# mcveanlab/mccortex

Hardware: AMD Instinct MI355X
Metric: k-mers/s inserted (build), k=31, 50M x 150bp synthetic reads (higher is better)
Workload: dtype u64

## Files before the change

### mccortex_amd/csrc/mcx_defer.h

```cpp
#pragma once
#include "mcx_kernels.h"

namespace mcx {

enum : int { BIN_OWNER = 0, BIN_GROUP = 1, BIN_SUBLOCAL = 2, BIN_GLOBAL = 3 };

struct BinSpec {
  int mode;
  uint32_t nparts;
  uint32_t nlocal;
  uint32_t rep;
  uint32_t nout;
  uint32_t seg_mod;
  uint32_t lb1;
  uint32_t region0;
};

__device__ __forceinline__ uint32_t out_seg(const BinSpec &bs, uint32_t ob0, uint32_t b)
{
  if (bs.mode == BIN_GLOBAL)
    return ((((b >> bs.lb1) * bs.rep + blockIdx.x % bs.rep) << bs.lb1) | (b & ((1u << bs.lb1) - 1u)));
  return ob0 + b;
}

struct BinOut {
  uint64_t *keys;
  uint8_t *edges;
  unsigned long long *counts;
  uint64_t cap;
  uint64_t *ov_keys;
  uint8_t *ov_edges;
  unsigned long long *ov_counts;
  uint64_t ov_cap;
};

#define MCX_LDS_AS __attribute__((address_space(3)))

#ifdef MCX_PHASES
__device__ unsigned long long g_phase[3][8];
#define MCX_PH_DECL unsigned long long ph_t = wall_clock64(), ph_acc[8] = {0, 0, 0, 0, 0, 0, 0, 0};
#define MCX_PH(i) { const unsigned long long n_ = wall_clock64(); ph_acc[i] += n_ - ph_t; ph_t = n_; }
#define MCX_PH_COUNT ph_acc[7]++;
#define MCX_PH_DUMP(kid) { if (threadIdx.x == 0) for (int i_ = 0; i_ < 8; i_++) atomicAdd(&g_phase[kid][i_], ph_acc[i_]); }
#else
#define MCX_PH_DECL
#define MCX_PH(i)
#define MCX_PH_COUNT
#define MCX_PH_DUMP(kid)
#endif
constexpr int kMaxBins = 2048;
constexpr uint64_t kQMask = (1ull << 56) - 1;

template <int W> __device__ __forceinline__ Kmer<W> tuple_pack(const Kmer<W> &q, uint32_t e)
{
  Kmer<W> t = q;
  t.w[0] |= (uint64_t)e << 56;
  return t;
}
template <int W> __device__ __forceinline__ Kmer<W> tuple_q(const Kmer<W> &t)
{
  Kmer<W> q = t;
  q.w[0] &= kQMask;
  return q;
}

constexpr int kRounds = 2;
constexpr int kStage = kTile / kRounds;

template <int T_, int TILE_, int R_ = kRounds> struct Geo {
  static constexpr int kT = T_, kTileG = TILE_, kRoundsG = R_, kStageG = TILE_ / R_;
};
using Geo256 = Geo<kThreads, kTile>;

template <int W, int NB, bool FULL, class G = Geo256> struct BinLds {
  using geo = G;
  uint64_t skey[G::kStageG * W];
  unsigned long long gbase[NB];
  uint32_t cnt[NB + 64];
  uint32_t rnk[NB + 64];
  uint32_t off[NB + 64];
  uint32_t wsum[G::kT / 64];
  uint16_t sbin[G::kStageG];
  uint8_t se[FULL ? G::kStageG : 16];
};

__device__ __forceinline__ uint32_t tid_now()
{
  uint32_t t = threadIdx.x;
  asm volatile("" : "+v"(t));
  return t;
}

template <int NB, int T = kThreads> struct BinRes { unsigned long long g0[(NB + T - 1) / T]; };

template <class LDS, int NB>
__device__ __forceinline__ void bin_reserve(LDS &L, const BinSpec &bs, const BinOut &out, uint32_t ob0, BinRes<NB, LDS::geo::kT> &res,
                                            bool trash_beyond = false)
{
  constexpr int kT = LDS::geo::kT;
  const int tid = threadIdx.x;
  __syncthreads();
  {
    constexpr int PERB = NB / kT;
    static_assert(NB % kT == 0, "bins per thread");
    uint32_t c[PERB], x = 0;
#pragma unroll
    for (int i = 0; i < PERB; i++) {
      const uint32_t b = (uint32_t)tid * PERB + i;
      c[i] = b < bs.nlocal ? L.cnt[b] : 0;
      x += c[i];
    }
    const uint32_t mine = x;
#pragma unroll
    for (int d = 1; d < 64; d <<= 1) {
      const uint32_t y = __shfl_up(x, d, 64);
      if ((tid & 63) >= d) x += y;
    }
    if ((tid & 63) == 63) L.wsum[tid >> 6] = x;
    __syncthreads();
    uint32_t before = 0, total = 0;
#pragma unroll
    for (int w = 0; w < kT / 64; w++) {
      const uint32_t ws = L.wsum[w];
      if (w < (tid >> 6)) before += ws;
      total += ws;
    }
    uint32_t o = before + x - mine;
#pragma unroll
    for (int i = 0; i < PERB; i++) {
      const uint32_t b = (uint32_t)tid * PERB + i;
      if (b < bs.nlocal) L.off[b] = o;
      o += c[i];
    }
    if (tid < 64) L.off[bs.nlocal + tid] = tid && trash_beyond ? (uint32_t)LDS::geo::kTileG : total;
  }
  __syncthreads();
#pragma unroll
  for (int q = 0; q < (NB + kT - 1) / kT; q++) {
    const uint32_t b = (uint32_t)q * kT + tid;
    res.g0[q] = 0;
    if (b < bs.nlocal) {
      const uint32_t c = L.cnt[b];
      if (c) res.g0[q] = atomicAdd(&out.counts[out_seg(bs, ob0, b)], (unsigned long long)c);
    }
  }
}

constexpr unsigned long long kDstMask = (1ULL << 48) - 1;

template <class LDS, int NB>
__device__ __forceinline__ void bin_commit(LDS &L, const BinSpec &bs, const BinOut &out, uint32_t ob0, const BinRes<NB, LDS::geo::kT> &res)
{
  constexpr int kT = LDS::geo::kT;
#pragma unroll
  for (int q = 0; q < (NB + kT - 1) / kT; q++) {
    const uint32_t b = (uint32_t)q * kT + threadIdx.x;
    if (b < bs.nlocal) {
      const uint32_t o0 = L.off[b], o1 = L.off[b + 1];
      const unsigned long long g0 = res.g0[q];
      const unsigned long long room = out.cap > g0 ? out.cap - g0 : 0;
      const uint32_t lim = o0 + (uint32_t)min((unsigned long long)(o1 - o0), room);
      const unsigned long long dst = ((unsigned long long)out_seg(bs, ob0, b) * out.cap + g0 - o0) & kDstMask;
      L.gbase[b] = dst | ((unsigned long long)lim << 48);
    }
  }
}

template <class LDS> __device__ __forceinline__ uint32_t bin_rank(LDS &L, uint32_t local)
{
  return L.off[local] + atomicAdd(&L.rnk[local], 1u);
}

template <int W, bool FULL, class LDS>
__device__ __forceinline__ void bin_place(LDS &L, int round, uint32_t p, uint32_t local, const Kmer<W> &t, uint32_t e)
{
  constexpr uint32_t kSt = LDS::geo::kStageG;
  if ((int)(p / kSt) != round) return;
  const uint32_t q = p % kSt;
  L.skey[q * W] = t.w[0];
  if (W == 2) L.skey[q * W + 1] = t.w[W - 1];
  L.sbin[q] = (uint16_t)local;
  if (FULL) L.se[q] = (uint8_t)e;
}

template <int W, bool ONECOL, bool FULL, int SH, class LDS>
__device__ __forceinline__ void bin_writeout(LDS &L, int round, const BinSpec &bs, const BinOut &out, uint32_t ob0,
                                             uint32_t region_of_seg, const InsertSink<W, ONECOL> &isink,
                                             uint32_t &novel, uint32_t &full)
{
  __syncthreads();
  const uint32_t n = L.off[bs.nlocal];
  constexpr uint32_t kSt = LDS::geo::kStageG;
  const uint32_t lo = (uint32_t)round * kSt;
  const uint32_t hi = min(n, lo + kSt);
  auto emit = [&](uint32_t p, uint32_t b, unsigned long long gb, uint64_t t0, uint64_t t1) {
    if (p < (uint32_t)(gb >> 48)) {
      const uint64_t at = (gb + p) & kDstMask;
      uint64_t *kd = out.keys + at * W;
      kd[0] = t0;
      if (W == 2) kd[1] = t1;
      if (FULL) out.edges[at] = L.se[p - lo];
    } else if (FULL || bs.mode == BIN_OWNER) {
      full = 2;
    } else {
      Kmer<W> tq;
      tq.w[0] = t0;
      if (W == 2) tq.w[W - 1] = t1;
      const uint32_t e = (uint32_t)(tq.w[0] >> 56);
      const Kmer<W> qq = tuple_q<W>(tq);
      const uint32_t lbq = lbq_of(isink.t);
      if (SH == 2) {
        const Kmer<W> key = key_unquot<W>(qq, lbq, b ^ mix_g(region_mix<W>(qq), lbq));
        const uint32_t owner = b >> bs.lb1;
        const unsigned long long pos = atomicAdd(&out.ov_counts[owner], 1ULL);
        if (pos < out.ov_cap) {
          uint64_t *kd = out.ov_keys + ((uint64_t)owner * out.ov_cap + pos) * W;
          kd[0] = key.w[0];
          if (W == 2) kd[1] = key.w[W - 1];
          out.ov_edges[(uint64_t)owner * out.ov_cap + pos] = (uint8_t)e;
        } else {
          const unsigned long long sp_cap = bs.region0 ? out.ov_counts[bs.nparts + 1] : 0;
          const unsigned long long sp = sp_cap ? atomicAdd(&out.ov_counts[bs.nparts], 1ULL) : 0;
          if (sp < sp_cap) {
            const uint64_t at = (uint64_t)bs.nparts * out.ov_cap + sp;
            uint64_t *kd = out.ov_keys + at * W;
            kd[0] = key.w[0];
            if (W == 2) kd[1] = key.w[W - 1];
            out.ov_edges[at] = (uint8_t)e;
          } else {
            full = 2;
          }
        }
      } else {
        table_mark_written(isink.t);
        table_count_fallback(isink.t);
        const uint32_t region = bs.mode == BIN_GROUP ? b : region_of_seg;
        const Kmer<W> key = key_unquot<W>(qq, lbq, r_of<W>(isink.t, region, qq));
        const uint64_t slot = key_slot<W>(isink.t, key);
        const uint64_t cur = *key_ptr_t<W, ONECOL>(isink.t, slot);
        probe_insert<W, ONECOL>(isink.t, key, slot, cur, 0, e, isink.col, novel, full);
      }
    }
  };
  for (uint32_t p = lo + threadIdx.x; p < hi; p += LDS::geo::kT) {
    const uint32_t q = p - lo;
    const uint32_t b = L.sbin[q];
    emit(p, b, L.gbase[b], L.skey[q * W], W == 2 ? L.skey[q * W + W - 1] : 0);
  }
  if (round + 1 < LDS::geo::kRoundsG) __syncthreads();
}

struct LaneWin { uint32_t a2, a1, a0, r2, r1, r0; };
__device__ __forceinline__ uint32_t pairrev32(uint32_t x)
{
  const uint32_t r = __builtin_bitreverse32(x);
  return ((r >> 1) & 0x55555555u) | ((r & 0x55555555u) << 1);
}
__device__ __forceinline__ LaneWin lane_win(const uint32_t *s_code, uint32_t pl, int k)
{
  LaneWin w;
  w.a2 = s_code[pl >> 4];
  w.a1 = s_code[(pl >> 4) + 1];
  w.a0 = s_code[(pl >> 4) + 2];
  const uint32_t c2 = pairrev32(~w.a0), c1 = pairrev32(~w.a1), c0 = pairrev32(~w.a2);
  const int t = 66 - 2 * k;
  if (t < 32) {
    w.r2 = (c2 << t) | (c1 >> (32 - t));
    w.r1 = (c1 << t) | (c0 >> (32 - t));
    w.r0 = c0 << t;
  } else {
    const uint64_t x = (((uint64_t)c1 << 32) | c0) << (t - 32);
    w.r2 = (uint32_t)(x >> 32);
    w.r1 = (uint32_t)x;
    w.r0 = 0;
  }
  return w;
}

template <int W, bool ONECOL>
__device__ __noinline__ void foreign_insert(const InsertSink<W, ONECOL> &isink, Kmer<W> key, uint32_t e,
                                            uint32_t &novel, uint32_t &full)
{
  table_mark_written(isink.t);
  table_count_foreign(isink.t);
  const uint64_t slot = key_slot<W>(isink.t, key);
  const uint64_t cur = *key_ptr_t<W, ONECOL>(isink.t, slot);
  probe_insert<W, ONECOL>(isink.t, key, slot, cur, 0, e, isink.col, novel, full);
}

template <int W, bool ONECOL, int NB, bool FULL, int SH, bool PK, int T = kThreads>
__global__ __launch_bounds__(T, (W == 1 ? 4 : 3)) void k_stream_bin(StreamArgs a_arg, BinSpec bs, BinOut out_arg,
                                                                  InsertSink<W, ONECOL> isink_arg)
{
  constexpr int H = T / kThreads;
  static_assert(T == kThreads || (T == 2 * kThreads && !FULL), "256 threads, or 512 for packed bins");
  __shared__ uint32_t s_code_h[H][kChunks + 4];
  __shared__ uint32_t s_inv_h[H][kChunks / 2 + 4];
  struct Cold { StreamArgs a; InsertSink<W, ONECOL> isink; };
  __shared__ Cold cold;
  if (threadIdx.x == 0) { cold.a = a_arg; cold.isink = isink_arg; }
  __syncthreads();
  const StreamArgs &a = cold.a;
  const BinOut &out = out_arg;
  const InsertSink<W, ONECOL> &isink = cold.isink;
  const uint64_t a_tile0 = a_arg.tile0, a_ntiles = a_arg.ntiles;
  const uint32_t t_lb1 = isink_arg.t.lb1, t_lbq = isink_arg.t.lb1 + isink_arg.t.lbo, t_part = isink_arg.t.part;
  extern __shared__ __attribute__((aligned(16))) unsigned char dyn_lds[];
  using LDS = BinLds<W, NB, FULL, Geo<T, T * kPosPerLane>>;
  LDS &L = *reinterpret_cast<LDS *>(dyn_lds);

  const int tid0 = threadIdx.x & (kThreads - 1);
  const uint64_t half0 = (uint64_t)(threadIdx.x / kThreads);
  const int k = a_arg.k;
  uint32_t n_kmers = 0, n_contigs = 0, n_novel = 0, full = 0;
  const uint64_t top_mask = (W == 1) ? (~0ULL >> (64 - 2 * k)) : (~0ULL >> (128 - 2 * k));
  const int first_shift = (W == 1) ? (2 * k - 2) : (2 * k - 66);
  const uint32_t ob0 = (blockIdx.x % bs.rep) * bs.nout;

  TileSrc pre;
  pre.a = make_uint4(0, 0, 0, 0); pre.b = make_uint4(0, 0, 0, 0);
  {
    const uint64_t t0 = a_tile0 + (uint64_t)blockIdx.x * H + half0;
    if (t0 < a_ntiles) tile_fetch<PK>(a_arg, t0, tid0, pre);
  }
  MCX_PH_DECL
  for (uint64_t tile_b = a_tile0 + (uint64_t)blockIdx.x * H; tile_b < a_ntiles; tile_b += (uint64_t)gridDim.x * H) {
    const int tid_blk = (int)tid_now();
    const int tid = tid_blk & (kThreads - 1);
    const uint64_t tile = tile_b + (uint64_t)(tid_blk / kThreads);
    const bool have_tile = H == 1 || tile < a_ntiles;
    uint32_t *s_code = s_code_h[H == 1 ? 0 : tid_blk / kThreads];
    uint32_t *s_inv = s_inv_h[H == 1 ? 0 : tid_blk / kThreads];
    MCX_PH(6) MCX_PH_COUNT
    tile_stage<PK>(a_arg, pre, tid, s_code, s_inv);
    for (uint32_t b = tid_blk; b < bs.nlocal + 64; b += T) { L.cnt[b] = 0; L.rnk[b] = 0; }
    if (tid < 4) { s_code[kChunks + tid] = 0; s_inv[kChunks / 2 + tid] = 0xFFFFFFFFu; }
    {
      const uint64_t tn = tile + (uint64_t)gridDim.x * H;
      if (tn < a_ntiles) tile_fetch<PK>(a_arg, tn, tid, pre);
    }
    __syncthreads();
    MCX_PH(0)

    const uint32_t pl = 16u * (uint32_t)(tid + 1);
    const uint64_t Vh = inv_win64(s_inv, pl);
    const uint64_t Vl = (W == 2) ? inv_win64(s_inv, pl + 64) : 0;
    const uint32_t prev_chunk_inv = (s_inv[(pl - 1) >> 5] >> (31 - ((pl - 1) & 31))) & 1u;
    uint32_t range = have_tile ? 0xFFFFu : 0u;
    if (have_tile) {
      const uint64_t plo = a.pos_lo, phi = a.pos_hi, T0 = tile * kTile;
      if (T0 < plo || T0 + kTile > phi) {
        const uint64_t P0 = T0 + 16ull * (uint64_t)tid;
        const int j_lo = plo > P0 ? (int)min((uint64_t)kPosPerLane, plo - P0) : 0;
        const int j_hi = phi > P0 ? (int)min((uint64_t)kPosPerLane, phi - P0) : 0;
        range = ((0x10000u >> j_lo) - 1u) & ~((0x10000u >> j_hi) - 1u);
      }
    }
    uint32_t ok16, nok16, pok16;
    {
      uint64_t Mh = Vh, Ml = Vl;
      for (int c = 1; c < k;) {
        const int s = min(c, k - c);
        if (W == 2) Mh |= (Mh << s) | (Ml >> (64 - s));
        else Mh |= Mh << s;
        if (W == 2) Ml |= Ml << s;
        c += s;
      }
      ok16 = ~(uint32_t)(Mh >> 48) & range;
      const int sh = 112 - k;
      const uint64_t nx = sh >= 64 ? (Vh >> (sh - 64)) : ((Vh << (64 - sh)) | (W == 2 ? (Vl >> sh) : 0));
      nok16 = ~(uint32_t)nx & 0xFFFFu;
      pok16 = ~((prev_chunk_inv << 15) | (uint32_t)(Vh >> 49)) & 0xFFFFu;
    }

    Kmer<W> tk[kPosPerLane];
    uint32_t tle[kPosPerLane];
    const uint32_t trash = bs.nlocal + 1u + ((uint32_t)tid_blk & 31u);
    n_kmers += __popc(ok16);
    n_contigs += __popc(ok16 & ~pok16);
    {
      const uint32_t own = s_code[pl >> 4];
      const uint32_t before = s_code[(pl - 1) >> 4] & 3u;
      const uint32_t lbq = t_lbq;
      const uint32_t qmask = (1u << lbq) - 1u, lmask = (1u << t_lb1) - 1u;
      Kmer<W> fw, rc;
      uint64_t feed;
      LaneWin lw;
      if (W == 1) {
        lw = lane_win(s_code, pl, k);
        feed = code_win64(s_code, pl + (uint32_t)k);
      } else {
        const uint64_t hi = code_win64(s_code, pl), lo = code_win64(s_code, pl + 32);
        const int s = 128 - 2 * k;
        fw.w[0] = hi >> s;
        fw.w[W - 1] = (lo >> s) | (hi << (64 - s));
        rc = revcomp<W>(fw, k);
        feed = code_win64(s_code, pl + (uint32_t)k);
      }
      const uint32_t feed32 = (uint32_t)(feed >> 32);
      uint32_t arr_prev = 0;
      const uint32_t key_sh = 64u - 2u * (uint32_t)k;
      const uint32_t mix_sh = (32u - lbq) & 31u;
#pragma unroll
      for (int j = 0; j < kPosPerLane; j++) {
        const uint32_t prev_nuc = j == 0 ? before : ((own >> (32 - 2 * j)) & 3u);
        const uint32_t nuc_next = (feed32 >> (30 - 2 * j)) & 3u;
        const uint32_t valid = 0u - ((ok16 >> (15 - j)) & 1u);
        const uint32_t nb = (nok16 >> (15 - j)) & 1u, pb = (pok16 >> (15 - j)) & 1u;
        uint32_t o, local;
        Kmer<W> key;
        uint64_t sel = 0;
        if (W == 1) {
          const uint32_t fh = j ? __builtin_amdgcn_alignbit(lw.a2, lw.a1, 32 - 2 * j) : lw.a2;
          const uint32_t fl = j ? __builtin_amdgcn_alignbit(lw.a1, lw.a0, 32 - 2 * j) : lw.a1;
          const uint32_t rh = j < 15 ? __builtin_amdgcn_alignbit(lw.r2, lw.r1, 2 + 2 * j) : lw.r2;
          const uint32_t rl = j < 15 ? __builtin_amdgcn_alignbit(lw.r1, lw.r0, 2 + 2 * j) : lw.r1;
          const uint64_t f = ((uint64_t)fh << 32) | fl, r = ((uint64_t)rh << 32) | rl;
          o = f < r ? 0u : 1u;
          sel = f < r ? f : r;
          key.w[0] = sel >> key_sh;
        } else {
          key = canonical<W>(fw, rc, o);
        }
        const uint32_t o4 = o << 2;
        const uint32_t e = (nb << (nuc_next | o4)) | (pb << ((prev_nuc ^ 7u) ^ o4));
        if (FULL) {
          uint32_t h2;
          kmer_hash<W>(key, 0, &h2);
          local = owner_of(h2, bs.nparts);
          tk[j] = key;
          local = (local & valid) | (trash & ~valid);
          tle[j] = local | (e << 24);
        } else {
          uint32_t G;
          Kmer<W> q;
          if (W == 1) {
            const uint64_t kk = sel >> key_sh;
            q.w[0] = kk >> lbq;
            G = ((uint32_t)kk ^ (region_mix<W>(q) >> mix_sh)) & qmask;
          } else {
            uint32_t r;
            q = key_quot<W>(key, lbq, r);
            G = r ^ mix_g(region_mix<W>(q), lbq);
          }
          local = SH == 1 ? (G & lmask) : G;
          tk[j] = tuple_pack<W>(q, e);
          if (SH == 1 && valid && (G >> t_lb1) != t_part) {
            foreign_insert<W, ONECOL>(isink, key, e, n_novel, full);
            local = trash;
          }
          local = (local & valid) | (trash & ~valid);
          tle[j] = local;
        }
        const uint32_t arr_now = atomicAdd(&L.cnt[local], 1u);
        if (j > 0) { tle[j - 1] |= arr_prev << 12; asm volatile("" : "+v"(tle[j - 1])); }
        arr_prev = arr_now;
        if (j == kPosPerLane - 1) tle[j] |= arr_now << 12;
        if (W == 1) asm volatile("" : "+v"(tle[j]), "+v"(tk[j].w[0]));
        else asm volatile("" : "+v"(tle[j]), "+v"(tk[j].w[0]), "+v"(tk[j].w[W - 1]));
        if (W == 2) {
          fw.w[0] = ((fw.w[0] << 2) | (fw.w[W - 1] >> 62)) & top_mask;
          fw.w[W - 1] = (fw.w[W - 1] << 2) | nuc_next;
          rc.w[W - 1] = (rc.w[W - 1] >> 2) | (rc.w[0] << 62);
          rc.w[0] = (rc.w[0] >> 2) | ((uint64_t)(3u - nuc_next) << first_shift);
        }
      }
    }
    MCX_PH(1)
    BinRes<NB, T> res;
    bin_reserve<LDS, NB>(L, bs, out, ob0, res, !FULL);
    MCX_PH(2)
#pragma unroll
    for (int j = 0; j < kPosPerLane; j++) {
      tle[j] += L.off[tle[j] & 0xfffu] << 12;
      if ((j & 3) == 3) asm volatile("" : "+v"(tle[j - 3]), "+v"(tle[j - 2]), "+v"(tle[j - 1]), "+v"(tle[j]));
    }
    bin_commit<LDS, NB>(L, bs, out, ob0, res);
    MCX_PH(3)
    for (int round = 0; round < kRounds; round++) {
#pragma unroll
      for (int j = 0; j < kPosPerLane; j++)
        bin_place<W, FULL, LDS>(L, round, FULL ? (tle[j] >> 12) & 0xfffu : tle[j] >> 12, tle[j] & 0xfffu, tk[j], tle[j] >> 24);
      bin_writeout<W, ONECOL, FULL, SH, LDS>(L, round, bs, out, ob0, 0, isink, n_novel, full);
      if (round == 0) { MCX_PH(4) } else { MCX_PH(5) }
    }
  }
  MCX_PH_DUMP(0)

  block_add(&a.ctr->kmers, n_kmers);
  block_add(&a.ctr->contigs, n_contigs);
  block_add(&a.ctr->novel, n_novel);
  if (full == 1) a.ctr->full = 1;
  if (full == 2) a.ctr->bin_over = 1;
  if (a.flag && n_contigs) *a.flag = 1;
}

struct TupleIn {
  const uint64_t *keys;
  const uint8_t *edges;
  const unsigned long long *counts;
  uint64_t seg_cap;
  uint32_t nseg;
  uint32_t seg_group, seg_stride;
  uint32_t set_rep;
  uint8_t set_map[32];
};
__device__ __forceinline__ uint64_t tuple_seg_phys(const TupleIn &in, uint32_t seg)
{
  uint32_t q = seg / in.seg_group;
  if (in.set_rep) q = (uint32_t)in.set_map[q / in.set_rep] * in.set_rep + q % in.set_rep;
  return (uint64_t)q * in.seg_stride + seg % in.seg_group;
}

template <int W, bool ONECOL, int NB, bool IN_FULL, bool SHARD, int T = kThreads, int R = kRounds, int P = 16>
__global__ __launch_bounds__(T, (W == 1 || T > kThreads ? 4 : 3)) void k_tuples_bin(TupleIn in, BinSpec bs, BinOut out,
                                                                         InsertSink<W, ONECOL> isink_arg, Counters *ctr)
{
  extern __shared__ __attribute__((aligned(16))) unsigned char dyn_lds[];
  using LDS = BinLds<W, NB, false, Geo<T, T * P, R>>;
  constexpr int kThreads = T, kTile = T * P;
  LDS &L = *reinterpret_cast<LDS *>(dyn_lds);
  __shared__ InsertSink<W, ONECOL> isink;
  if (threadIdx.x == 0) isink = isink_arg;
  __syncthreads();
  const uint32_t t_spb = isink_arg.t.spb, t_lb1 = isink_arg.t.lb1, t_lbq = isink_arg.t.lb1 + isink_arg.t.lbo, t_part = isink_arg.t.part;
  const int tid = threadIdx.x;
  uint32_t n_novel = 0, full = 0;
  const uint64_t chunks_per_seg = (in.seg_cap + kTile - 1) / kTile;
  const bool xcd = bs.mode == BIN_SUBLOCAL && gridDim.x % 8 == 0 && bs.seg_mod % 8 == 0 && in.nseg % bs.seg_mod == 0;
  const uint32_t group = xcd ? blockIdx.x % 8 : 0;
  const uint32_t nseg_g = xcd ? in.nseg / 8 : in.nseg;
  constexpr uint32_t kWin = 2;
  const uint32_t bins_g = xcd ? bs.seg_mod / 8 : 1;
  const uint32_t reps = xcd ? in.nseg / bs.seg_mod : 1;
  const uint32_t win_segs = kWin * reps;
  const uint32_t nwin = (bins_g + kWin - 1) / kWin;
  const uint64_t nchunks = xcd ? (uint64_t)nwin * chunks_per_seg * win_segs : chunks_per_seg * nseg_g;
  const uint64_t v0 = xcd ? blockIdx.x / 8 : blockIdx.x, vstep = xcd ? gridDim.x / 8 : gridDim.x;
  const uint32_t lmask = (1u << t_lb1) - 1u;
  MCX_PH_DECL
  for (uint64_t v = v0; v < nchunks; v += vstep) {
    uint32_t seg;
    uint64_t start;
    if (xcd) {
      const uint64_t per_win = chunks_per_seg * win_segs;
      const uint32_t win = (uint32_t)(v / per_win);
      const uint64_t rem = v % per_win;
      const uint32_t s = (uint32_t)(rem % win_segs);
      const uint32_t rgi = win * kWin + s % kWin;
      if (rgi >= bins_g) continue;
      seg = (s / kWin) * bs.seg_mod + group + 8 * rgi;
      start = (rem / win_segs) * kTile;
    } else {
      seg = (uint32_t)(v % nseg_g);
      start = (v / nseg_g) * kTile;
    }
    const uint64_t pseg = tuple_seg_phys(in, seg);
    uint64_t cnt = in.counts ? (uint64_t)in.counts[pseg] : in.seg_cap;
    if (cnt > in.seg_cap) cnt = in.seg_cap;
    if (start >= cnt) continue;
    const uint32_t n = (uint32_t)min((uint64_t)kTile, cnt - start);
    const uint32_t lregion = bs.mode == BIN_SUBLOCAL ? seg % bs.seg_mod : 0;
    const uint32_t region = bs.region0 + lregion;
    const uint32_t ob0 = (bs.mode == BIN_SUBLOCAL ? lregion * t_spb : 0) + (blockIdx.x % bs.rep) * bs.nout;
    MCX_PH(6) MCX_PH_COUNT
    __syncthreads();
    for (uint32_t b = tid; b < bs.nlocal + 64; b += kThreads) { L.cnt[b] = 0; L.rnk[b] = 0; }
    __syncthreads();
    MCX_PH(0)
    const uint32_t trash = bs.nlocal + 1u + ((uint32_t)tid & 31u);
    const uint64_t *kin = in.keys + (pseg * in.seg_cap + start) * W;
    const uint8_t *ein = IN_FULL ? in.edges + pseg * in.seg_cap + start : nullptr;
    constexpr int PER = kTile / kThreads;
    Kmer<W> tk[PER];
    uint32_t ev[IN_FULL ? PER : 1], loc[PER];
    uint32_t okm = 0;
    const bool vec16 = !IN_FULL && (((uintptr_t)in.keys & 15u) == 0) && (W == 2 || (in.seg_cap & 1u) == 0);
    if (vec16) {
      const ulonglong2 *kin2 = reinterpret_cast<const ulonglong2 *>(kin);
#pragma unroll
      for (int q = 0; q < PER; q += (W == 1 ? 2 : 1)) {
        const uint32_t p = (uint32_t)(q / (W == 1 ? 2 : 1)) * kThreads + tid;
        const uint32_t i = W == 1 ? 2 * p : p;
        tk[q].w[0] = 0; tk[q + (W == 1 ? 1 : 0)].w[W - 1] = 0;
        if (i < n) {
          const ulonglong2 x = kin2[p];
          okm |= 1u << q;
          if (W == 1) {
            tk[q].w[0] = x.x;
            tk[q + (W == 1 ? 1 : 0)].w[0] = x.y;
            if (i + 1 < n) okm |= 2u << q;
          } else {
            tk[q].w[0] = x.x;
            tk[q].w[W - 1] = x.y;
          }
        }
      }
    } else {
#pragma unroll
    for (int q = 0; q < PER; q++) {
      const uint32_t i = (uint32_t)q * kThreads + tid;
      if (i < n) okm |= 1u << q;
      tk[q].w[0] = 0; if (W == 2) tk[q].w[W - 1] = 0;
      if (IN_FULL) ev[q] = 0;
      if (i < n) {
        tk[q].w[0] = kin[(uint64_t)i * W];
        if (W == 2) tk[q].w[W - 1] = kin[(uint64_t)i * W + 1];
        if (IN_FULL) ev[q] = ein[i];
      }
    }
    }
#pragma unroll
    for (int q = 0; q < PER; q++) {
      const uint32_t i = (uint32_t)q * kThreads + tid;
      uint32_t hb;
      if (IN_FULL) {
        uint32_t r;
        const uint32_t lbq = t_lbq;
        const Kmer<W> key = tk[q];
        const Kmer<W> qq = key_quot<W>(key, lbq, r);
        const uint32_t G = r ^ mix_g(region_mix<W>(qq), lbq);
        hb = 0;
        loc[q] = G & lmask;
// ... 436 lines not shown
```

### mccortex_amd/csrc/mcx_kernels.h

```cpp
#pragma once
#include <hip/hip_runtime.h>
#include <stdint.h>
#include "mcx_kmer.h"

namespace mcx {

constexpr int kBucket = 4;
template <int W> struct Sub {
  static constexpr int kShift = W == 1 ? 12 : 11;
  static constexpr uint64_t kSlots = 1ull << kShift;
  static constexpr uint32_t kBuckets = (uint32_t)(kSlots / kBucket);
};
__host__ __device__ constexpr int sub_shift_for_words(int W) { return W == 1 ? 12 : 11; }

struct TableView {
  uint64_t *rec;
  uint64_t nslots;
  uint64_t nmain;
  uint32_t lb1;
  uint32_t lbo;
  uint32_t part;
  uint32_t spb;
  uint32_t S;
  uint32_t max_probe;
// ... 389 lines not shown
      if (cv) __hip_atomic_fetch_add(val, (uint64_t)cv << 8, MCX_RLX, MCX_AGENT);
      if (e) __hip_atomic_fetch_or(val, (uint64_t)e, MCX_RLX, MCX_AGENT);
    }
    loaded++;
  }
  if (novel) { atomicAdd(&ctr->novel, (unsigned long long)novel); atomicAdd(&st->novel, (unsigned long long)novel); }
  if (loaded) atomicAdd(&st->loaded, (unsigned long long)loaded);
  if (full) ctr->full = 1;
}

template <int W>
__global__ __launch_bounds__(256) void k_record_keys(const uint8_t *recs, uint64_t n, uint32_t rec_bytes, uint64_t *k0, uint64_t *k1)
{
  const uint64_t i = (uint64_t)blockIdx.x * blockDim.x + threadIdx.x;
  if (i >= n) return;
  const uint8_t *p = recs + i * rec_bytes;
  k0[i] = (uint64_t)load_le32(p) | (uint64_t)load_le32(p + 4) << 32;
  if (W == 2) k1[i] = (uint64_t)load_le32(p + 8) | (uint64_t)load_le32(p + 12) << 32;
}

__global__ __launch_bounds__(256) void k_gather_records(const uint8_t *in, const uint64_t *perm, uint64_t n, uint32_t rec_bytes, uint8_t *out)
{
  const uint64_t i = ((uint64_t)blockIdx.x * blockDim.x + threadIdx.x) >> 4;
  const uint32_t l = threadIdx.x & 15u;
  if (i >= n) return;
  const uint8_t *src = in + perm[i] * rec_bytes;
  uint8_t *dst = out + i * rec_bytes;
  for (uint32_t b = l; b < rec_bytes; b += 16) dst[b] = src[b];
}

template <int W>
__global__ __launch_bounds__(256) void k_check_sorted(const uint64_t *k0, const uint64_t *k1, uint64_t n, unsigned long long *first_bad)
{
  const uint64_t i = (uint64_t)blockIdx.x * blockDim.x + threadIdx.x;
  if (i + 1 >= n) return;
  bool lt = k0[i] < k0[i + 1];
  if (W == 2 && k0[i] == k0[i + 1]) lt = k1[i] < k1[i + 1];
  if (!lt) atomicMin(first_bad, (unsigned long long)(i + 1));
}

__global__ __launch_bounds__(256) void k_covg_scan(TableView t, uint32_t ncols, unsigned long long *out,
                                                   unsigned long long *hist, uint32_t nbins, uint32_t lbins)
{
  extern __shared__ unsigned long long s_acc[];
  unsigned long long *s_hist = s_acc + 2 * ncols;
  for (uint32_t c = threadIdx.x; c < 2 * ncols + lbins; c += blockDim.x) s_acc[c] = 0;
  __syncthreads();
  for (uint64_t slot = (uint64_t)blockIdx.x * blockDim.x + threadIdx.x; slot < t.nslots; slot += (uint64_t)gridDim.x * blockDim.x) {
    const uint64_t *r = key_ptr(t, slot);
    uint64_t w0, v1 = 0;
    if (t.S == 2) {
      const ulonglong2 kv = *reinterpret_cast<const ulonglong2 *>(r);
      w0 = kv.x; v1 = kv.y;
    } else {
      w0 = r[0];
    }
    if (!(w0 & kFlag)) continue;
    uint64_t sum = 0;
    for (uint32_t c = 0; c < ncols; c++) {
      uint64_t cv = (t.S == 2 ? v1 : *val_ptr(t, slot, c)) >> 8;
      if (cv > 0xFFFFFFFFull) cv = 0xFFFFFFFFull;
      if (cv) { atomicAdd(&s_acc[c], 1ULL); atomicAdd(&s_acc[ncols + c], (unsigned long long)cv); }
      sum += cv;
    }
    if (sum > 0xFFFFFFFFull) sum = 0xFFFFFFFFull;
    if (hist) {
      const uint64_t bin = sum < nbins ? sum : nbins - 1;
      if (bin < lbins) atomicAdd(&s_hist[bin], 1ULL);
      else atomicAdd(&hist[bin], 1ULL);
    }
  }
  __syncthreads();
  for (uint32_t c = threadIdx.x; c < 2 * ncols; c += blockDim.x)
    if (s_acc[c]) atomicAdd(&out[c], s_acc[c]);
  for (uint32_t c = threadIdx.x; c < lbins; c += blockDim.x)
    if (s_hist[c]) atomicAdd(&hist[c], s_hist[c]);
}

template <int W, bool ONECOL> struct InsertSink {
  TableView t;
  uint32_t col;
};

constexpr int kThreads = 256;
constexpr int kPosPerLane = 16;
constexpr int kTile = kThreads * kPosPerLane;
constexpr int kChunks = 272;
constexpr int kBatch = 4;

struct StreamArgs {
  const uint8_t *stream;
  const uint32_t *code;
  const uint16_t *inv;
  uint64_t nbytes;
  uint64_t pos_lo, pos_hi;
  uint64_t tile0, ntiles;
  int k;
  Counters *ctr;
  unsigned char *flag;
};

__device__ __forceinline__ uint64_t code_win64(const uint32_t *s_code, uint32_t q)
{
  const uint32_t j = q >> 4, sh = (q & 15u) * 2u;
  const uint64_t hi = ((uint64_t)s_code[j] << 32) | s_code[j + 1];
  const uint64_t lo = s_code[j + 2];
  return sh ? (hi << sh) | (lo >> (32 - sh)) : hi;
}
__device__ __forceinline__ uint64_t inv_win64(const uint32_t *s_inv, uint32_t q)
{
  const uint32_t j = q >> 5, sh = q & 31u;
  const uint64_t hi = ((uint64_t)s_inv[j] << 32) | s_inv[j + 1];
  const uint64_t lo = s_inv[j + 2];
  return sh ? (hi << sh) | (lo >> (32 - sh)) : hi;
}

__device__ __forceinline__ uint4 load_chunk(const uint8_t *stream, uint64_t nbytes, int64_t g)
{
  if (g >= 0 && (uint64_t)g + 16 <= nbytes) return *reinterpret_cast<const uint4 *>(stream + g);
  uint32_t w[4] = {0, 0, 0, 0};
  if (g + 16 > 0 && g < (int64_t)nbytes)
    for (int i = 0; i < 16; i++) {
      const int64_t p = g + i;
      if (p >= 0 && (uint64_t)p < nbytes) w[i >> 2] |= (uint32_t)stream[p] << (8 * (i & 3));
    }
  return make_uint4(w[0], w[1], w[2], w[3]);
}

__device__ __forceinline__ void encode_words(const uint4 v, uint32_t &code, uint32_t &inv)
{
  const uint32_t w[4] = {v.x, v.y, v.z, v.w};
  code = 0; inv = 0;
#pragma unroll
  for (int i = 0; i < 4; i++) {
    const uint32_t x = w[i];
    const uint32_t t = ((x >> 1) ^ (x >> 2)) & 0x03030303u;
    code = (code << 8) | ((t * 0x40100401u) >> 24);
    const uint32_t u = x & 0xDFDFDFDFu;
#define MCX_NZ(v) ((((v) & 0x7F7F7F7Fu) + 0x7F7F7F7Fu) | (v))
    const uint32_t bad = MCX_NZ(u ^ 0x41414141u) & MCX_NZ(u ^ 0x43434343u) &
                         MCX_NZ(u ^ 0x47474747u) & MCX_NZ(u ^ 0x54545454u) & 0x80808080u;
#undef MCX_NZ
    inv = (inv << 4) | ((((bad >> 7) * 0x08040201u) >> 24) & 0xFu);
  }
}

__device__ __forceinline__ void encode_chunk(const uint8_t *stream, uint64_t nbytes, int64_t g,
                                             uint32_t &code, uint32_t &inv)
{
  encode_words(load_chunk(stream, nbytes, g), code, inv);
}

struct TileSrc { uint4 a, b; };
template <bool PK> __device__ __forceinline__ void tile_fetch(const StreamArgs &a, uint64_t tile, int tid, TileSrc &t)
{
  if (PK) {
    const int64_t c0 = (int64_t)(tile * (kTile / 16)) - 1;
    const int64_t nch = (int64_t)((a.nbytes + 15) / 16);
    const int64_t c = c0 + tid, c2 = c + kThreads;
    const bool in = c >= 0 && c < nch;
    t.a.x = in ? a.code[c] : 0u;
    t.a.y = in ? (uint32_t)a.inv[c] : 0xFFFFu;
    if (tid < kChunks - kThreads) {
      const bool in2 = c2 >= 0 && c2 < nch;
      t.b.x = in2 ? a.code[c2] : 0u;
      t.b.y = in2 ? (uint32_t)a.inv[c2] : 0xFFFFu;
    }
  } else {
    const int64_t r0 = (int64_t)(tile * kTile) - 16;
    t.a = load_chunk(a.stream, a.nbytes, r0 + 16 * (int64_t)tid);
    if (tid < kChunks - kThreads) t.b = load_chunk(a.stream, a.nbytes, r0 + 16 * (int64_t)(tid + kThreads));
  }
}
template <bool PK> __device__ __forceinline__ void tile_stage(const StreamArgs &a, const TileSrc &t, int tid, uint32_t *s_code, uint32_t *s_inv)
{
  uint32_t code, inv;
  (void)a;
  if (PK) { code = t.a.x; inv = t.a.y; } else encode_words(t.a, code, inv);
  s_code[tid] = code;
  reinterpret_cast<uint16_t *>(s_inv)[tid ^ 1] = (uint16_t)inv;
  if (tid < kChunks - kThreads) {
    if (PK) { code = t.b.x; inv = t.b.y; } else encode_words(t.b, code, inv);
    s_code[tid + kThreads] = code;
    reinterpret_cast<uint16_t *>(s_inv)[(tid + kThreads) ^ 1] = (uint16_t)inv;
  }
}

__global__ void k_pack_stream(const uint8_t *stream, uint64_t nbytes, uint32_t *code_out, uint16_t *inv_out)
{
  const uint64_t c = (uint64_t)blockIdx.x * blockDim.x + threadIdx.x;
  if (c * 16 >= nbytes) return;
  uint32_t code, inv;
  encode_words(load_chunk(stream, nbytes, (int64_t)(c * 16)), code, inv);
  code_out[c] = code;
  inv_out[c] = (uint16_t)inv;
}

template <int W> struct Occ {
  Kmer<W> key;
  uint32_t e;
};

template <int W, bool ONECOL>
__device__ __forceinline__ void flush_batch(const InsertSink<W, ONECOL> &sink, const Occ<W> (&occ)[kBatch],
                                            const bool (&ov)[kBatch], uint32_t &novel, uint32_t &full)
{
  uint64_t slot[kBatch], cur[kBatch], hint[kBatch];
#pragma unroll
  for (int i = 0; i < kBatch; i++) {
    cur[i] = 0; hint[i] = 0; slot[i] = 0;
    if (ov[i]) {
      slot[i] = key_slot<W>(sink.t, occ[i].key);
      const uint64_t *r = key_ptr_t<W, ONECOL>(sink.t, slot[i]);
      if (W == 1 && ONECOL) {
        const ulonglong2 kv = *reinterpret_cast<const ulonglong2 *>(r);
        cur[i] = kv.x; hint[i] = kv.y;
      } else {
        cur[i] = r[0];
      }
    }
  }
#pragma unroll
  for (int i = 0; i < kBatch; i++)
    if (ov[i]) probe_insert<W, ONECOL>(sink.t, occ[i].key, slot[i], cur[i], hint[i], occ[i].e, sink.col, novel, full);
}

__device__ __forceinline__ uint32_t owner_of(uint32_t h2, uint32_t nparts)
{
  return (uint32_t)(((uint64_t)h2 * nparts) >> 32);
}

__device__ __forceinline__ void lane_masks_wide(const uint32_t *s_inv, uint32_t pl, int k, uint32_t &ok16, uint32_t &nok16)
{
  const uint64_t V0 = inv_win64(s_inv, pl), V1 = inv_win64(s_inv, pl + 64), V2 = inv_win64(s_inv, pl + 128);
  uint64_t M0 = V0, M1 = V1, M2 = V2;
  for (int c = 1; c < k;) {
    const int s = min(c, k - c);
    if (s < 64) {
      M0 |= (M0 << s) | (M1 >> (64 - s));
      M1 |= (M1 << s) | (M2 >> (64 - s));
      M2 |= M2 << s;
    } else {
      const int t = s - 64;
      M0 |= t ? (M1 << t) | (M2 >> (64 - t)) : M1;
      M1 |= M2 << t;
    }
    c += s;
  }
  ok16 = ~(uint32_t)(M0 >> 48) & 0xFFFFu;
  const int wi = k >> 6, sh = k & 63;
  const uint64_t a = wi == 0 ? V0 : V1, b = wi == 0 ? V1 : V2;
  const uint64_t nx = sh ? (a << sh) | (b >> (64 - sh)) : a;
  nok16 = ~(uint32_t)(nx >> 48) & 0xFFFFu;
}

template <int W, bool ONECOL, bool PK>
__global__ __launch_bounds__(kThreads, 1) void k_stream(StreamArgs a, InsertSink<W, ONECOL> isink)
{
  if (blockIdx.x == 0 && threadIdx.x == 0) table_mark_written(isink.t);
  __shared__ uint32_t s_code[kChunks + 4];
  __shared__ uint32_t s_inv[kChunks / 2 + 4];

  const int tid = threadIdx.x;
  const int k = a.k;
  uint32_t n_kmers = 0, n_contigs = 0, n_novel = 0, full = 0;

  const uint64_t top_mask = ~0ULL >> (64 * W - 2 * k);
  const int first_shift = 2 * k - 2 - 64 * (W - 1);

  for (uint64_t tile = a.tile0 + blockIdx.x; tile < a.ntiles; tile += gridDim.x) {
    __syncthreads();
    {
      TileSrc ts;
      tile_fetch<PK>(a, tile, tid, ts);
      tile_stage<PK>(a, ts, tid, s_code, s_inv);
    }
    if (tid < 4) { s_code[kChunks + tid] = 0; s_inv[kChunks / 2 + tid] = 0xFFFFFFFFu; }
    __syncthreads();

    const uint32_t pl = 16u * (uint32_t)(tid + 1);
    const uint64_t Vh = inv_win64(s_inv, pl);
    const uint32_t prev_chunk_inv = (s_inv[(pl - 1) >> 5] >> (31 - ((pl - 1) & 31))) & 1u;

    const uint64_t P0 = tile * kTile + 16ull * (uint64_t)tid;
    const int j_lo = a.pos_lo > P0 ? (int)min((uint64_t)kPosPerLane, a.pos_lo - P0) : 0;
    const int j_hi = a.pos_hi > P0 ? (int)min((uint64_t)kPosPerLane, a.pos_hi - P0) : 0;

    if constexpr (W > 2) {
      uint32_t ok16, nok16;
      lane_masks_wide(s_inv, pl, k, ok16, nok16);
      ok16 &= ((0x10000u >> j_lo) - 1u) & ~((0x10000u >> j_hi) - 1u);
      const uint32_t pok16 = ~((prev_chunk_inv << 15) | (uint32_t)(Vh >> 49)) & 0xFFFFu;
      Occ<W> occ[kBatch];
      bool ov[kBatch];
      if (ok16) {
        Kmer<W> fw, rc;
        const int topb = k - 32 * (W - 1);
        fw.w[0] = code_win64(s_code, pl) >> (64 - 2 * topb);
        for (int i = 1; i < W; i++) fw.w[i] = code_win64(s_code, pl + (uint32_t)(topb + 32 * (i - 1)));
        rc = revcomp<W>(fw, k);
        const uint64_t feed = code_win64(s_code, pl + (uint32_t)k);
        const int fs = 2 * topb - 2;
        uint32_t prev_nuc = s_code[(pl - 1) >> 4] & 3u;
#pragma unroll
        for (int j = 0; j < kPosPerLane; j++) {
          const bool valid = (ok16 >> (15 - j)) & 1u;
          const bool next_ok = (nok16 >> (15 - j)) & 1u, prev_ok = (pok16 >> (15 - j)) & 1u;
          const uint32_t nuc_next = (uint32_t)(feed >> (62 - 2 * j)) & 3u;
          ov[j % kBatch] = valid;
          if (valid) {
            uint32_t o;
            Occ<W> &x = occ[j % kBatch];
            x.key = canonical<W>(fw, rc, o);
            uint32_t e = 0;
            if (next_ok) e |= 1u << (nuc_next + 4u * o);
            if (prev_ok) e |= 1u << ((3u - prev_nuc) + 4u * (1u - o));
            x.e = e;
            n_kmers++;
            n_contigs += prev_ok ? 0u : 1u;
          }
          if (j % kBatch == kBatch - 1) flush_batch<W, ONECOL>(isink, occ, ov, n_novel, full);
          prev_nuc = kmer_first_base<W>(fw, k);
          kmer_push<W>(fw, nuc_next, k);
          for (int i = W - 1; i >= 1; i--) rc.w[i] = (rc.w[i] >> 2) | (rc.w[i - 1] << 62);
          rc.w[0] = (rc.w[0] >> 2) | ((uint64_t)(3u - nuc_next) << fs);
        }
      }
      continue;
    }
    const uint64_t Vl = (W == 2) ? inv_win64(s_inv, pl + 64) : 0;
    bool any = false;
#pragma unroll
    for (int j = 0; j < kPosPerLane; j++) {
      const uint64_t Th = (W == 2 && j) ? ((Vh << j) | (Vl >> (64 - j))) : (Vh << j);
      any |= ((Th >> (64 - k)) == 0) & (j >= j_lo) & (j < j_hi);
    }

    Occ<W> occ[kBatch];
// ... 555 lines not shown
```

Before: 104.5 billion.

## Compact live chunks per half-block in 512-thread stream bin kernel

For the two-half (512-thread) variant, each half now walks its own contiguous chunk range through a larger sliding window. Chunks whose k-mer windows would all be invalidated by non-ACGT bytes are dropped, and the surviving chunks are compacted into a live list with ballot and mbcnt so that every lane processes a useful chunk. The window then advances by however many live chunks were consumed, which is meant to avoid wasting lanes on dead positions. In exchange it adds extra LDS state, a data-dependent advance, and another barrier and compaction step per iteration. The 256-thread path is unchanged.

```diff
diff --git a/mccortex_amd/csrc/mcx_defer.h b/mccortex_amd/csrc/mcx_defer.h
--- a/mccortex_amd/csrc/mcx_defer.h
+++ b/mccortex_amd/csrc/mcx_defer.h
@@ -95,10 +95,10 @@
 
 template <class LDS, int NB>
 __device__ __forceinline__ void bin_reserve(LDS &L, const BinSpec &bs, const BinOut &out, uint32_t ob0, BinRes<NB, LDS::geo::kT> &res,
-                                            bool trash_beyond = false)
+                                            bool trash_beyond = false, int tid_opaque = -1)
 {
   constexpr int kT = LDS::geo::kT;
-  const int tid = threadIdx.x;
+  const int tid = tid_opaque < 0 ? (int)threadIdx.x : tid_opaque;
   __syncthreads();
   {
     constexpr int PERB = NB / kT;
@@ -288,16 +288,37 @@
   probe_insert<W, ONECOL>(isink.t, key, slot, cur, 0, e, isink.col, novel, full);
 }
 
+constexpr int kLiveWin = 288;
+constexpr int kLiveChunks = kLiveWin + 16;
+__device__ __forceinline__ uint64_t uniform64(uint64_t x)
+{
+  return ((uint64_t)__builtin_amdgcn_readfirstlane((uint32_t)(x >> 32)) << 32) | __builtin_amdgcn_readfirstlane((uint32_t)x);
+}
+
 template <int W, bool ONECOL, int NB, bool FULL, int SH, bool PK, int T = kThreads>
 __global__ __launch_bounds__(T, (W == 1 ? 4 : 3)) void k_stream_bin(StreamArgs a_arg, BinSpec bs, BinOut out_arg,
                                                                   InsertSink<W, ONECOL> isink_arg)
 {
   constexpr int H = T / kThreads;
-  static_assert(T == kThreads || (T == 2 * kThreads && !FULL), "256 threads, or 512 for packed bins");
-  __shared__ uint32_t s_code_h[H][kChunks + 4];
-  __shared__ uint32_t s_inv_h[H][kChunks / 2 + 4];
+  constexpr bool LIVE = H == 2;
+  constexpr int NCH = LIVE ? kLiveChunks : kChunks;
+  static_assert(T == kThreads || (T == 2 * kThreads && !FULL && W == 1), "256 threads, or 512 for packed one-word bins");
+  __shared__ uint32_t s_code_h[H][NCH + 4];
+  __shared__ uint32_t s_inv_h[H][NCH / 2 + 4];
+  struct LiveHalf { uint64_t cur, end; uint32_t more, nlive[5]; uint16_t live[5 * 64]; };
+  __shared__ LiveHalf s_lh[2];
   struct Cold { StreamArgs a; InsertSink<W, ONECOL> isink; };
   __shared__ Cold cold;
+  const int tid0 = threadIdx.x & (kThreads - 1);
+  const uint64_t half0 = (uint64_t)(threadIdx.x / kThreads);
+  uint64_t cur0 = 0, cend0 = 0;
+  if constexpr (LIVE) {
+    const uint64_t cb = a_arg.pos_lo / 16, ce = (a_arg.pos_hi + 15) / 16;
+    const uint64_t units = (uint64_t)gridDim.x * H, per = (ce - cb + units - 1) / units;
+    cur0 = min(cb + ((uint64_t)blockIdx.x * H + half0) * per, ce);
+    cend0 = min(cur0 + per, ce);
+    if (tid0 == 0) { s_lh[half0].cur = cur0; s_lh[half0].end = cend0; s_lh[half0].more = cur0 < cend0; }
+  }
   if (threadIdx.x == 0) { cold.a = a_arg; cold.isink = isink_arg; }
   __syncthreads();
   const StreamArgs &a = cold.a;
@@ -309,8 +330,6 @@
   using LDS = BinLds<W, NB, FULL, Geo<T, T * kPosPerLane>>;
   LDS &L = *reinterpret_cast<LDS *>(dyn_lds);
 
-  const int tid0 = threadIdx.x & (kThreads - 1);
-  const uint64_t half0 = (uint64_t)(threadIdx.x / kThreads);
   const int k = a_arg.k;
   uint32_t n_kmers = 0, n_contigs = 0, n_novel = 0, full = 0;
   const uint64_t top_mask = (W == 1) ? (~0ULL >> (64 - 2 * k)) : (~0ULL >> (128 - 2 * k));
@@ -319,35 +338,93 @@
 
   TileSrc pre;
   pre.a = make_uint4(0, 0, 0, 0); pre.b = make_uint4(0, 0, 0, 0);
-  {
-    const uint64_t t0 = a_tile0 + (uint64_t)blockIdx.x * H + half0;
+  if constexpr (LIVE) {
+    if (cur0 < cend0) win_fetch<PK, NCH>(a_arg, (int64_t)cur0 - 1, tid0, pre);
+  } else {
+    const uint64_t t0 = a_tile0 + (uint64_t)blockIdx.x;
     if (t0 < a_ntiles) tile_fetch<PK>(a_arg, t0, tid0, pre);
   }
   MCX_PH_DECL
-  for (uint64_t tile_b = a_tile0 + (uint64_t)blockIdx.x * H; tile_b < a_ntiles; tile_b += (uint64_t)gridDim.x * H) {
+  for (uint64_t tile_b = a_tile0 + (uint64_t)blockIdx.x; LIVE || tile_b < a_ntiles; tile_b += (uint64_t)gridDim.x) {
+    if constexpr (LIVE) { if (!__builtin_amdgcn_readfirstlane(s_lh[0].more | s_lh[1].more)) break; }
     const int tid_blk = (int)tid_now();
     const int tid = tid_blk & (kThreads - 1);
     const uint64_t tile = tile_b + (uint64_t)(tid_blk / kThreads);
-    const bool have_tile = H == 1 || tile < a_ntiles;
     uint32_t *s_code = s_code_h[H == 1 ? 0 : tid_blk / kThreads];
     uint32_t *s_inv = s_inv_h[H == 1 ? 0 : tid_blk / kThreads];
     MCX_PH(6) MCX_PH_COUNT
-    tile_stage<PK>(a_arg, pre, tid, s_code, s_inv);
-    for (uint32_t b = tid_blk; b < bs.nlocal + 64; b += T) { L.cnt[b] = 0; L.rnk[b] = 0; }
-    if (tid < 4) { s_code[kChunks + tid] = 0; s_inv[kChunks / 2 + tid] = 0xFFFFFFFFu; }
-    {
-      const uint64_t tn = tile + (uint64_t)gridDim.x * H;
-      if (tn < a_ntiles) tile_fetch<PK>(a_arg, tn, tid, pre);
-    }
-    __syncthreads();
+    uint32_t pl, range;
+    if constexpr (LIVE) {
+      LiveHalf &lh = s_lh[tid_blk / kThreads];
+      const uint64_t cur = uniform64(lh.cur), left64 = uniform64(lh.end) - cur;
+      const uint32_t left = (left64 >> 32) ? 0xFFFFFFFFu : (uint32_t)left64;
+      uint32_t inv_a, inv_b;
+      win_stage<PK, NCH>(pre, tid, s_code, s_inv, inv_a, inv_b);
+      for (uint32_t b = tid_blk; b < bs.nlocal + 64; b += T) { L.cnt[b] = 0; L.rnk[b] = 0; }
+      if (tid < 4) { s_code[NCH + tid] = 0; s_inv[NCH / 2 + tid] = 0xFFFFFFFFu; }
+      {
+        const uint32_t nrem = min(left, (uint32_t)kLiveWin);
+        const uint32_t m0 = k >= 16 ? 1u : 0u, m1 = k >= 17 ? (0xFFFFu << (32 - k)) & 0xFFFFu : 0u;
+        const uint32_t lane = (uint32_t)tid & 63u, wv = (uint32_t)tid >> 6;
+        uint32_t nx_a = (uint32_t)__builtin_amdgcn_ds_bpermute((tid + 1) << 2, (int)inv_a);
+        if (lane == 63u) nx_a = 0;
+        const bool live_a = tid >= 1 && (uint32_t)tid <= nrem && !((inv_a & m0) | (nx_a & m1));
+        const unsigned long long bal_a = __ballot(live_a);
+        const uint32_t rk_a = __builtin_amdgcn_mbcnt_hi((uint32_t)(bal_a >> 32), __builtin_amdgcn_mbcnt_lo((uint32_t)bal_a, 0u));
+        if (live_a) lh.live[wv * 64u + rk_a] = (uint16_t)tid;
+        if (lane == 0) lh.nlive[wv] = (uint32_t)__popcll(bal_a);
+        if (wv == 0) {
+          const uint32_t nx_b = (uint32_t)__builtin_amdgcn_ds_bpermute((tid + 1) << 2, (int)inv_b);
+          const bool live_b = (uint32_t)tid + kThreads <= nrem && !((inv_b & m0) | (nx_b & m1));
+          const unsigned long long bal_b = __ballot(live_b);
+          const uint32_t rk_b = __builtin_amdgcn_mbcnt_hi((uint32_t)(bal_b >> 32), __builtin_amdgcn_mbcnt_lo((uint32_t)bal_b, 0u));
+          if (live_b) lh.live[4 * 64u + rk_b] = (uint16_t)(tid + kThreads);
+          if (lane == 0) lh.nlive[4] = (uint32_t)__popcll(bal_b);
+        }
+      }
+      __syncthreads();
+      const uint32_t b1 = lh.nlive[0], b2 = b1 + lh.nlive[1], b3 = b2 + lh.nlive[2], b4 = b3 + lh.nlive[3], nl = b4 + lh.nlive[4];
+      auto nth_live = [&](uint32_t r) -> uint32_t {
+        const uint32_t seg = (r >= b1) + (r >= b2) + (r >= b3) + (r >= b4);
+        const uint32_t base = r >= b4 ? b4 : r >= b3 ? b3 : r >= b2 ? b2 : r >= b1 ? b1 : 0u;
+        return lh.live[seg * 64u + (r - base)];
+      };
+      const bool have = (uint32_t)tid < nl;
+      const uint32_t sc = have ? nth_live((uint32_t)tid) : 1u;
+      const uint32_t adv = __builtin_amdgcn_readfirstlane(nl > (uint32_t)kThreads ? nth_live(kThreads - 1) : (uint32_t)kLiveWin);
+      const bool more = adv < left;
+      const uint64_t cnext = cur + min(adv, left);
+      if (more) win_fetch<PK, NCH>(a_arg, (int64_t)cnext - 1, tid, pre);
+      if (tid == 0) { lh.cur = cnext; lh.more = more; }
+      pl = 16u * sc;
+      range = have ? 0xFFFFu : 0u;
+      {
+        const uint64_t plo = a.pos_lo, phi = a.pos_hi, W0 = cur * 16;
+        if (W0 < plo || W0 + 16ull * kLiveWin > phi) {
+          const uint64_t P0 = W0 + 16ull * (uint64_t)(sc - 1u);
+          const int j_lo = plo > P0 ? (int)min((uint64_t)kPosPerLane, plo - P0) : 0;
+          const int j_hi = phi > P0 ? (int)min((uint64_t)kPosPerLane, phi - P0) : 0;
+          range &= ((0x10000u >> j_lo) - 1u) & ~((0x10000u >> j_hi) - 1u);
+        }
+      }
+    } else {
+      tile_stage<PK>(a_arg, pre, tid, s_code, s_inv);
+      for (uint32_t b = tid_blk; b < bs.nlocal + 64; b += T) { L.cnt[b] = 0; L.rnk[b] = 0; }
+      if (tid < 4) { s_code[kChunks + tid] = 0; s_inv[kChunks / 2 + tid] = 0xFFFFFFFFu; }
+      {
+        const uint64_t tn = tile + (uint64_t)gridDim.x;
+        if (tn < a_ntiles) tile_fetch<PK>(a_arg, tn, tid, pre);
+      }
+      __syncthreads();
+      pl = 16u * (uint32_t)(tid + 1);
+    }
     MCX_PH(0)
 
-    const uint32_t pl = 16u * (uint32_t)(tid + 1);
     const uint64_t Vh = inv_win64(s_inv, pl);
     const uint64_t Vl = (W == 2) ? inv_win64(s_inv, pl + 64) : 0;
     const uint32_t prev_chunk_inv = (s_inv[(pl - 1) >> 5] >> (31 - ((pl - 1) & 31))) & 1u;
-    uint32_t range = have_tile ? 0xFFFFu : 0u;
-    if (have_tile) {
+    if constexpr (!LIVE) {
+      range = 0xFFFFu;
       const uint64_t plo = a.pos_lo, phi = a.pos_hi, T0 = tile * kTile;
       if (T0 < plo || T0 + kTile > phi) {
         const uint64_t P0 = T0 + 16ull * (uint64_t)tid;
@@ -468,7 +545,7 @@
     }
     MCX_PH(1)
     BinRes<NB, T> res;
-    bin_reserve<LDS, NB>(L, bs, out, ob0, res, !FULL);
+    bin_reserve<LDS, NB>(L, bs, out, ob0, res, !FULL, LIVE ? tid_blk : -1);
     MCX_PH(2)
 #pragma unroll
     for (int j = 0; j < kPosPerLane; j++) {
diff --git a/mccortex_amd/csrc/mcx_kernels.h b/mccortex_amd/csrc/mcx_kernels.h
--- a/mccortex_amd/csrc/mcx_kernels.h
+++ b/mccortex_amd/csrc/mcx_kernels.h
@@ -565,38 +565,49 @@
 }
 
 struct TileSrc { uint4 a, b; };
-template <bool PK> __device__ __forceinline__ void tile_fetch(const StreamArgs &a, uint64_t tile, int tid, TileSrc &t)
-{
+template <bool PK, int NCH> __device__ __forceinline__ void win_fetch(const StreamArgs &a, int64_t c0, int tid, TileSrc &t)
+{
+  static_assert(NCH > kThreads && NCH <= 2 * kThreads, "two chunks per thread at most");
   if (PK) {
-    const int64_t c0 = (int64_t)(tile * (kTile / 16)) - 1;
     const int64_t nch = (int64_t)((a.nbytes + 15) / 16);
     const int64_t c = c0 + tid, c2 = c + kThreads;
     const bool in = c >= 0 && c < nch;
     t.a.x = in ? a.code[c] : 0u;
     t.a.y = in ? (uint32_t)a.inv[c] : 0xFFFFu;
-    if (tid < kChunks - kThreads) {
+    if (tid < NCH - kThreads) {
       const bool in2 = c2 >= 0 && c2 < nch;
       t.b.x = in2 ? a.code[c2] : 0u;
       t.b.y = in2 ? (uint32_t)a.inv[c2] : 0xFFFFu;
     }
   } else {
-    const int64_t r0 = (int64_t)(tile * kTile) - 16;
+    const int64_t r0 = c0 * 16;
     t.a = load_chunk(a.stream, a.nbytes, r0 + 16 * (int64_t)tid);
-    if (tid < kChunks - kThreads) t.b = load_chunk(a.stream, a.nbytes, r0 + 16 * (int64_t)(tid + kThreads));
-  }
+    if (tid < NCH - kThreads) t.b = load_chunk(a.stream, a.nbytes, r0 + 16 * (int64_t)(tid + kThreads));
+  }
+}
+template <bool PK, int NCH>
+__device__ __forceinline__ void win_stage(const TileSrc &t, int tid, uint32_t *s_code, uint32_t *s_inv, uint32_t &inv_a, uint32_t &inv_b)
+{
+  uint32_t code;
+  if (PK) { code = t.a.x; inv_a = t.a.y; } else encode_words(t.a, code, inv_a);
+  s_code[tid] = code;
+  reinterpret_cast<uint16_t *>(s_inv)[tid ^ 1] = (uint16_t)inv_a;
+  inv_b = 0;
+  if (tid < NCH - kThreads) {
+    if (PK) { code = t.b.x; inv_b = t.b.y; } else encode_words(t.b, code, inv_b);
+    s_code[tid + kThreads] = code;
+    reinterpret_cast<uint16_t *>(s_inv)[(tid + kThreads) ^ 1] = (uint16_t)inv_b;
+  }
+}
+template <bool PK> __device__ __forceinline__ void tile_fetch(const StreamArgs &a, uint64_t tile, int tid, TileSrc &t)
+{
+  win_fetch<PK, kChunks>(a, (int64_t)(tile * (kTile / 16)) - 1, tid, t);
 }
 template <bool PK> __device__ __forceinline__ void tile_stage(const StreamArgs &a, const TileSrc &t, int tid, uint32_t *s_code, uint32_t *s_inv)
 {
-  uint32_t code, inv;
+  uint32_t ia, ib;
   (void)a;
-  if (PK) { code = t.a.x; inv = t.a.y; } else encode_words(t.a, code, inv);
-  s_code[tid] = code;
-  reinterpret_cast<uint16_t *>(s_inv)[tid ^ 1] = (uint16_t)inv;
-  if (tid < kChunks - kThreads) {
-    if (PK) { code = t.b.x; inv = t.b.y; } else encode_words(t.b, code, inv);
-    s_code[tid + kThreads] = code;
-    reinterpret_cast<uint16_t *>(s_inv)[(tid + kThreads) ^ 1] = (uint16_t)inv;
-  }
+  win_stage<PK, kChunks>(t, tid, s_code, s_inv, ia, ib);
 }
 
 __global__ void k_pack_stream(const uint8_t *stream, uint64_t nbytes, uint32_t *code_out, uint16_t *inv_out)
```

Measured after the change: 102.9 billion. 0.984x the previous value.
